# tphakala/birdnet-go

Measured on AMD Instinct MI355X. Metric: 3s-48kHz clips/sec (whole node) + max-abs prob diff vs TFLite, BirdNET v2.4, higher is better.
Workload: dtype f32; 1 GPU; BASELINE configs[1]: BirdNET v2.4 fp32, batch 256 x 3 s @ 48 kHz per GPU, mel front-end + CNN + head on device, raw logits out; batch_per_gpu=256, n_samples=144000, n_classes=6522, pipeline_depth=2, input_sets=4

## Files before the change

### birdnet-go_amd/csrc/engine.cpp

```cpp
#include "engine.h"

#include <algorithm>
#include <cmath>
#include <cstdio>
#include <cstdlib>
#include <cstring>
#include <mutex>
#include <sstream>

#include "../../include/bnhip.h"
#include "hostpipe.h"

namespace bnhip {

#define HIPCHK(call)                                                                           \
    do {                                                                                       \
        hipError_t e_ = (call);                                                                \
        if (e_ != hipSuccess) {                                                                \
            *err = std::string(#call) + ": " + hipGetErrorString(e_);                          \
            return false;                                                                      \
        }                                                                                      \
    } while (0)

Engine::~Engine() {
// ... 154 lines not shown
    return t;
}
bool Engine::tail_taken(int si, int n, bool lane_tuning) const {
    const Step& s = steps[si];
    if (s.kind != S_PW || !s.tail || !s.wbx) return false;
    const int wm = lane_tuning ? s.wm : s.wm_full, nt = lane_tuning ? s.nt : s.nt_full;
    if (wm < 13) return false;
    const int last = si + (s.tail == 1 ? 2 : 1), s_end = part_s1 < 0 ? (int)steps.size() : part_s1;
    if (si < part_s0 || last >= s_end) return false;
    if (s.tail == 2 && steps[si + 1].dwl) return false;
    const PwParams p = pw_params(s, n, lane_tuning);
    if (!pw_tail_ok(p, tail_of(s, steps[si + 1]), nt, wm)) return false;
    return (pw_sw & PW_SW_TAIL_FORCE) || pw_tail_fills(p, nt, wm);
}

float* Engine::vptr(int v, const float* d_in, float* d_logits, float* d_emb, int lane) const {
    if (v < 0) return nullptr;
    if (v == v_input) return const_cast<float*>(d_in);
    if (v == v_logits) return d_logits;
    if (part_hand && v == v_hand) return part_hand;
    (void)d_emb;
    char* base = cur_arena ? cur_arena : act_arena;
    if (lane >= 0) return reinterpret_cast<float*>(base + (size_t)lane * lane_bytes + vals[v].offset_lane);
    return reinterpret_cast<float*>(base + vals[v].offset);
}

hipEvent_t Engine::get_event() {
    if (!ev_pool.empty()) { hipEvent_t e = ev_pool.back(); ev_pool.pop_back(); return e; }
    hipEvent_t e; hipEventCreate(&e); return e;
}
// ... 8 lines not shown
    if (depth <= 1 || (profiling && profile_filter.empty())) return run(d_in, n, d_logits, d_emb, err);
    const int c = (int)(call_idx++ % (unsigned)depth);
    if (ctx_stream[c] != stream) {
        hipEventRecord(ev_ctx_fork, stream);
        hipStreamWaitEvent(ctx_stream[c], ev_ctx_fork, 0);
    }
    cur_arena = ctx_arena[c];
    cur_stream = ctx_stream[c];
    cur_ctx = c;
    bool ok = run_eager(d_in, n, d_logits, d_emb, err);
    cur_arena = nullptr;
    cur_stream = nullptr;
    cur_ctx = -1;
    return ok;
}
bool Engine::run_on_context(int c, hipStream_t st, const float* d_in, int n, float* d_logits, float* d_emb, std::string* err) {
    if (n <= 0 || n > max_batch) { *err = "batch size out of range"; return false; }
    if (c < 0 || c >= kMaxDepth || !st || !ctx_arena[c]) { *err = "context does not exist"; return false; }
    call_idx++;
    cur_arena = ctx_arena[c];
    cur_stream = st;
    cur_ctx = c;
    bool ok = run_eager(d_in, n, d_logits, d_emb, err);
    cur_ctx = -1;
    cur_arena = nullptr;
    cur_stream = nullptr;
    return ok;
}
bool Engine::run_part(int c, hipStream_t st, int s0, int s1, const float* d_in, int n, float* hand, float* d_logits, float* d_emb, std::string* err) {
    if (n <= 0 || n > max_batch) { *err = "batch size out of range"; return false; }
    if (c < 0 || c >= kMaxDepth || !st || !ctx_arena[c]) { *err = "context does not exist"; return false; }
    if (v_hand < 0 || !hand || s0 < 0 || s1 > (int)steps.size() || s0 >= s1 || (s0 != 0 && s0 != split_step) || (s1 != (int)steps.size() && s1 != split_step)) {
        *err = "not a cut of this plan"; return false;
    }
    call_idx++;
    cur_arena = ctx_arena[c];
    cur_stream = st;
    cur_ctx = c;
    part_s0 = s0; part_s1 = s1; part_hand = hand;
    bool ok = run_eager(d_in, n, d_logits, d_emb, err);
    part_s0 = 0; part_s1 = -1; part_hand = nullptr;
    cur_ctx = -1;
    cur_arena = nullptr;
    cur_stream = nullptr;
    return ok;
}
int Engine::heatmap_pruned_step() const {
    if (steps.empty() || precision != 0) return -1;
    const Step& s = steps.back();
    if (s.kind != S_PW || s.out != v_logits || s.in1 >= 0 || s.in2 >= 0 || s.H * s.W != 1 || s.Co != n_classes) return -1;
    if (s.in0 < 0 || vals[s.in0].half || vals[s.in0].elems != (size_t)s.C) return -1;
    return (int)steps.size() - 1;
}
bool Engine::run_head(int s1, const float* d_in, int n, std::string* err) {
    if (n <= 0 || n > max_batch) { *err = "batch size out of range"; return false; }
// ... 40 lines not shown
        }
    }
    if (pick < 0) return;
    split_step = pick; v_hand = crossing[pick];
    if (getenv("BNHIP_DEBUG")) {
        fprintf(stderr, "[bnhip] host split: step %d (%s), value %d (%zu elems/clip%s); candidates:", split_step, steps[split_step].name.c_str(), v_hand,
                vals[v_hand].elems, vals[v_hand].half ? ", bf16" : "");
        for (int k : split_candidates) fprintf(stderr, " %d", k);
        fprintf(stderr, "\n");
    }
}
void Engine::sync_contexts() {
    for (int i = 0; i < kMaxKStreams; i++) if (kstream[i]) hipStreamSynchronize(kstream[i]);
}

bool Engine::run(const float* d_in, int n, float* d_logits, float* d_emb, std::string* err) {
    if (n <= 0 || n > max_batch) { *err = "batch size out of range"; return false; }
    if (call_idx) {
        for (int c = 0; c < kMaxDepth; c++)
            if (ctx_stream[c] && ctx_stream[c] != stream) { hipEventRecord(ev_ctx_done[c], ctx_stream[c]); hipStreamWaitEvent(stream, ev_ctx_done[c], 0); }
        if (kstream[0] && kstream[0] != stream) hipStreamSynchronize(kstream[0]);
    }
    if (!use_graphs || profiling) return run_eager(d_in, n, d_logits, d_emb, err);
    GraphEntry* ge = nullptr;
    for (auto& g : graphs)
        if (g.in == d_in && g.logits == d_logits && g.emb == d_emb && g.n == n) { ge = &g; break; }
    if (ge && ge->exec) {
        hipError_t e = hipGraphLaunch(ge->exec, stream);
        if (e != hipSuccess) { *err = std::string("hipGraphLaunch: ") + hipGetErrorString(e); return false; }
        return true;
    }
    if (!ge) {
        if (graphs.size() >= 8) { if (graphs.front().exec) hipGraphExecDestroy(graphs.front().exec); graphs.erase(graphs.begin()); }
        graphs.push_back(GraphEntry{d_in, d_logits, d_emb, n, 1, nullptr});
        return run_eager(d_in, n, d_logits, d_emb, err);
    }
    hipGraph_t graph = nullptr;
    hipError_t e = hipStreamBeginCapture(stream, hipStreamCaptureModeRelaxed);
    if (e != hipSuccess) { (void)hipGetLastError(); use_graphs = false; return run_eager(d_in, n, d_logits, d_emb, err); }
    bool ok = run_eager(d_in, n, d_logits, d_emb, err);
    e = hipStreamEndCapture(stream, &graph);
    if (!ok || e != hipSuccess || !graph) {
        if (graph) hipGraphDestroy(graph);
        (void)hipGetLastError();
        use_graphs = false;
        return run_eager(d_in, n, d_logits, d_emb, err);
    }
    hipGraphExec_t exec = nullptr;
    e = hipGraphInstantiate(&exec, graph, nullptr, nullptr, 0);
    hipGraphDestroy(graph);
    if (e != hipSuccess || !exec) { (void)hipGetLastError(); use_graphs = false; return run_eager(d_in, n, d_logits, d_emb, err); }
    ge->exec = exec;
    e = hipGraphLaunch(exec, stream);
    if (e != hipSuccess) { *err = std::string("hipGraphLaunch: ") + hipGetErrorString(e); return false; }
    return true;
}

bool Engine::run_eager(const float* d_in_all, int n_all, float* d_logits_all, float* d_emb_all, std::string* err) {
    struct Lane { const float* d_in; int n; float* d_logits; float* d_emb; hipStream_t st; int clip0; };
    Lane lanes[kMaxLanes];
    int nl = 1;
    hipStream_t main_stream = cur_stream ? cur_stream : stream;
    if (mm_dirty) {
        for (int i = 0; i < kMaxKStreams; i++) if (kstream[i]) hipStreamSynchronize(kstream[i]);
        if (stream) hipStreamSynchronize(stream);
        if (mm_scratch) hipMemset(mm_scratch, 0, (size_t)kMaxDepth * kMaxLanes * kMinMaxScratch * sizeof(float));
        (void)hipGetLastError();
        mm_dirty = false;
    }
    if (n_lanes > 1 && !cur_stream && (!profiling || !profile_filter.empty()) && n_all >= dual_lane_min) nl = std::min(n_lanes, n_all);
    for (int li = 0, c0 = 0; li < nl; li++) {
        int cnt = n_all / nl + (li < n_all % nl ? 1 : 0);
        lanes[li] = Lane{d_in_all + (size_t)c0 * n_samples, cnt, d_logits_all + (size_t)c0 * n_classes,
                         d_emb_all ? d_emb_all + (size_t)c0 * emb_dim : nullptr, li == 0 ? main_stream : lane_stream[li - 1], c0};
        c0 += cnt;
    }
    hipEvent_t st_a = nullptr, st_b = nullptr;
    if (step_timing) { hipEventCreate(&st_a); hipEventCreate(&st_b); hipEventRecord(st_a, main_stream); }
    if (nl > 1) {
        hipEventRecord(ev_fork, main_stream);
        for (int li = 1; li < nl; li++) hipStreamWaitEvent(lanes[li].st, ev_fork, 0);
    }
    const int s_end = part_s1 < 0 ? (int)steps.size() : part_s1;
    for (int si = part_s0; si < s_end; si++) {
      for (int li = 0; li < nl; li++) {
        const Step& s = steps[si];
        const float* d_in = lanes[li].d_in; float* d_logits = lanes[li].d_logits; float* d_emb = lanes[li].d_emb;
        const int n = lanes[li].n, clip0 = nl > 1 ? li : -1;
        hipStream_t stream = lanes[li].st;
        float* in0 = vptr(s.in0, d_in, d_logits, d_emb, clip0);
        float* in1 = vptr(s.in1, d_in, d_logits, d_emb, clip0);
        float* in2 = vptr(s.in2, d_in, d_logits, d_emb, clip0);
        float* out = vptr(s.out, d_in, d_logits, d_emb, clip0);
        float* out2 = vptr(s.out2, d_in, d_logits, d_emb, clip0);
        if (s.kind == S_DW && si > 0 && steps[si - 1].tail == 2 && tail_taken(si - 1, n, nl > 1)) continue;
        if (s.kind == S_MEAN_PARTIAL && si > 0 && steps[si - 1].tail == 1 && tail_taken(si - 1, n, nl > 1)) continue;
        if (s.kind == S_MEAN_FINISH && si > 1 && steps[si - 2].tail == 1 && tail_taken(si - 2, n, nl > 1)) continue;
        ProfEntry pe{};
        static const char* dbg_sync_before = getenv("BNHIP_DEBUG_SYNC_BEFORE");
        static const char* dbg_sync_after = getenv("BNHIP_DEBUG_SYNC_AFTER");
        static const char* dbg_ctx1_only = getenv("BNHIP_DEBUG_CTX1_ONLY");
        if (dbg_ctx1_only && cur_ctx == 1 && !strstr(dbg_ctx1_only, s.kclass)) continue;
        static const char* dbg_ctx1_skip = getenv("BNHIP_DEBUG_CTX1_SKIP");
        if (dbg_ctx1_skip && cur_ctx == 1 && strstr(dbg_ctx1_skip, s.kclass)) continue;
        if (dbg_sync_before && (!strcmp(dbg_sync_before, s.kclass) || s.name.rfind(dbg_sync_before, 0) == 0)) hipStreamSynchronize(stream);
        const bool prof_this = profiling && (profile_filter.empty() || profile_filter == s.kclass);
        if (prof_this) { pe.a = get_event(); pe.b = get_event(); pe.step = si; pe.n = n; hipEventRecord(pe.a, stream); }
        switch (s.kind) {
            case S_MINMAX:
                launch_clip_minmax(in0, n, n_samples, specs[0].eps, reinterpret_cast<float2*>(out),
                                   mm_scratch ? mm_scratch + ((size_t)std::max(cur_ctx, 0) * kMaxLanes + (size_t)li) * kMinMaxScratch : nullptr, stream);
                break;
            case S_FRONTEND: {
                const FrontSpec& fs = specs[s.spec];
                FrontendParams p;
                p.x = in0; p.mm = reinterpret_cast<const float2*>(in1); p.G = fs.G; p.window = fs.window; p.out = out;
                p.n_samples = n_samples; p.L = fs.L; p.Lfft = fs.Lfft; p.Kp = fs.Kp; p.hop = fs.hop; p.F = fs.F; p.n_mels = fs.n_mels;
                p.NTP = fs.NTP; p.C = C_spec; p.c = fs.c; p.norm_sub = fs.norm_sub; p.norm_mul = fs.norm_mul;
                p.p1 = fs.p1; p.p2 = fs.p2; p.n_clips = n;
                launch_frontend(p, stream);
                break;
            }
            case S_NORMALIZE:
                launch_normalize(in0, reinterpret_cast<const float2*>(in1), out, n, n_samples, specs[0].norm_sub, specs[0].norm_mul, stream);
// ... 225 lines not shown
}

std::string Engine::profile_read() {
    hipStreamSynchronize(stream);
    struct Agg { double ms = 0, flops = 0, bytes = 0; long launches = 0; };
    std::map<std::string, Agg> agg;
    std::vector<std::string> order;
    std::vector<Agg> per_step(steps.size());
    for (auto& e : prof) {
        float ms = 0;
        hipEventElapsedTime(&ms, e.a, e.b);
        const Step& s = steps[e.step];
        const StepView sv = step_view(*this, e.step);
        if (!agg.count(s.kclass)) order.push_back(s.kclass);
        Agg& a = agg[s.kclass];
        a.ms += ms; a.launches++; a.flops += sv.flops * e.n; a.bytes += sv.bytes * e.n + s.wbytes;
        Agg& ps = per_step[e.step];
        ps.ms += ms; ps.launches++; ps.flops += sv.flops * e.n; ps.bytes += sv.bytes * e.n + s.wbytes;
        ev_pool.push_back(e.a); ev_pool.push_back(e.b);
    }
    prof.clear();
    std::ostringstream os;
    os << "[";
    for (size_t i = 0; i < order.size(); i++) {
        const Agg& a = agg[order[i]];
        os << (i ? "," : "") << "{\"kernel\":\"" << order[i] << "\",\"launches\":" << a.launches << ",\"ms\":" << a.ms
           << ",\"flops\":" << a.flops << ",\"bytes\":" << a.bytes << "}";
    }
    for (size_t i = 0; i < steps.size(); i++) {
        const Agg& a = per_step[i];
        if (!a.launches) continue;
        os << ",{\"step\":" << i << ",\"kernel\":\"" << steps[i].kclass << "\",\"name\":\"";
        jesc(os, step_view(*this, i).name);
// ... 8 lines not shown
```

### birdnet-go_amd/csrc/engine.h

```cpp
#pragma once
#include <hip/hip_runtime.h>

#include <map>
#include <string>
#include <vector>

#include "kernels.h"
#include "tflite_model.h"

namespace bnhip {

enum StepKind { S_MINMAX, S_FRONTEND, S_NORMALIZE, S_STFT, S_MELFIN, S_MELBAND, S_CONV_DIRECT, S_PW, S_DW, S_EXPAND_DW, S_MEAN_PARTIAL, S_MEAN_FINISH, S_SE, S_UNARY, S_BINARY,
                S_EW_UNARY, S_EW_BINARY, S_POOL, S_COPY, S_SOFTMAX, S_REDUCE, S_CONV_GENERIC,
                S_CONV_IGEMM };

struct GenGeom {
    int d[4] = {1, 1, 1, 1};
    long sa[4] = {0, 0, 0, 0}, sb[4] = {0, 0, 0, 0}, so[4] = {0, 0, 0, 0};
    long offa = 0, offo = 0;
    bool a_const = false, b_const = false;
    int mask = 0;
    float alpha = 0.f;
    bool fill = false;
    int dh = 1, dw = 1, depthwise = 0, mult = 1;
// ... 34 lines not shown
    int L, Kp, Lfft, hop, F, n_mels, NTP, c;
    float p1, p2, eps, norm_sub, norm_mul;
    const double* G = nullptr;
    const float* window = nullptr;
    bool fft = false;
    int nb = 0, nbp = 0, mode = 0;
    const float* window_full = nullptr;
    const double* stft_tw = nullptr;
    unsigned stft_zmask = 0xffffffffu;
    const int* bins = nullptr;
    bool normalize = true, log_compress = false, time_major = false;
    int pad_left = 0;
    float log_floor = 0.f, log_scale = 1.f;
};

struct ProfEntry { hipEvent_t a, b; int step; int n; };

struct WeightPlan {
    std::vector<float> img;
    std::vector<size_t> step_w[4];
    std::vector<size_t> step_bx;
};

inline DwParams dw_params(const Step& s, const float* in = nullptr, float* out = nullptr, int n = 1) {
    return DwParams{in, s.w0, s.w1, out, n, s.H, s.W, s.C, s.Ho, s.Wo, s.kh, s.kw, s.sh, s.sw, s.pt, s.pl, s.act};
}
PwTail tail_of(const Step& s, const Step& c);

class Engine {
  public:
    ~Engine();
    bool build(TflModel m, int device, int max_batch, bool plan_only, std::string* err, int* code);
    bool run(const float* d_in, int n, float* d_logits, float* d_emb, std::string* err);

    int device = 0, max_batch = 256;
    bool no_reuse = false;
    bool autotune = true;
    bool defer_weights = false;
    void finish_deferred();
    char* weights_ptr() const { return w_arena; }
    size_t weights_bytes() const { return w_bytes; }
    int frontend_fft = -1;
    int logits_output = -1, embedding_output = -2;
    int precision = 0;
    int bf16x3 = 0;
    int pw_sw = 0;
    bool use_graphs = false;
    void drop_graphs();
    static constexpr int kMaxDepth = 3;
    int depth = 1;
    hipStream_t ctx_stream[kMaxDepth] = {nullptr, nullptr, nullptr};
    char* ctx_arena[kMaxDepth] = {nullptr, nullptr, nullptr};
    static constexpr int kMinMaxScratch = 16 * (2 * kMinMaxParts + 2);
    float* mm_scratch = nullptr;
    bool mm_dirty = false;
    hipEvent_t ev_ctx_fork = nullptr, ev_ctx_done[kMaxDepth] = {nullptr, nullptr, nullptr};
    unsigned call_idx = 0;
    bool run_pipelined(const float* d_in, int n, float* d_logits, float* d_emb, std::string* err);
    void sync_contexts();
    int host_depth = 2;
    bool ensure_contexts(int d, std::string* err, bool with_streams = true);
    bool run_on_context(int c, hipStream_t st, const float* d_in, int n, float* d_logits, float* d_emb, std::string* err);
    int split_step = -1, v_hand = -1;
    float* d_hand = nullptr;
    std::vector<int> split_candidates;
    void pick_split();
    size_t hand_clip_bytes() const { return v_hand < 0 ? 0 : vals[v_hand].elems * (vals[v_hand].half ? 2 : 4); }
    bool ensure_hand(std::string* err);
    bool run_part(int c, hipStream_t st, int s0, int s1, const float* d_in, int n, float* hand, float* d_logits, float* d_emb, std::string* err);
    int heatmap_pruned_step() const;
    bool run_head(int s1, const float* d_in, int n, std::string* err);
    struct HostPipe* hostpipe = nullptr;
    static constexpr int kMaxLanes = 4;
    int n_lanes = 2;
    int dual_lane_min = 32;
    hipStream_t lane_stream[kMaxLanes - 1] = {nullptr, nullptr, nullptr};
    hipEvent_t ev_fork = nullptr, ev_join[kMaxLanes - 1] = {nullptr, nullptr, nullptr};
    void mark_tails();
    bool tail_taken(int si, int n, bool lane_tuning) const;
    PwParams pw_params(const Step& s, int n, bool lane_tuning) const;
    void mark_bf16_storage();
    void tune_or_load();
    void autotune_pw();
    void autotune_expdw();
// ... 34 lines not shown
    float* d_stage_emb = nullptr;
    int16_t* d_stage_pcm = nullptr;
    size_t stage_pcm_bytes = 0;
    float* d_post_conf = nullptr;
    float* d_topk_conf = nullptr;
    int32_t* d_topk_idx = nullptr;
    int topk_cap = 0;

    std::string describe() const;
    std::string profile_read();
    bool step_timing = false;
    std::vector<std::pair<hipEvent_t, hipEvent_t>> step_ev;
    int steps_read(double* start_ms, double* end_ms, int cap);

  private:
    struct GraphEntry { const float* in; float* logits; float* emb; int n; int seen; hipGraphExec_t exec; };
    std::vector<GraphEntry> graphs;
    bool run_eager(const float* d_in, int n, float* d_logits, float* d_emb, std::string* err);
    char* act_arena = nullptr;
    char* cur_arena = nullptr;
    hipStream_t cur_stream = nullptr;
    int cur_ctx = -1;
    int part_s0 = 0, part_s1 = -1;
    float* part_hand = nullptr;
    size_t act_bytes = 0;
    char* w_arena = nullptr;
    size_t w_bytes = 0;
    std::vector<ProfEntry> prof;
    std::vector<hipEvent_t> ev_pool;
    float* vptr(int v, const float* d_in, float* d_logits, float* d_emb, int lane = -1) const;
    int lane_cap = 0;
    size_t lane_bytes = 0;
    hipEvent_t get_event();
// ... 5 lines not shown
```

### birdnet-go_amd/csrc/frontend.hip

```cpp
#include "kernels.h"

#include <cmath>
#include <cstdlib>

namespace bnhip {

__global__ void k_pcm16_to_f32(const int16_t* __restrict__ pcm, float* __restrict__ out, size_t n) {
    size_t i = (size_t)blockIdx.x * blockDim.x + threadIdx.x;
    size_t stride = (size_t)gridDim.x * blockDim.x;
    for (; i < n; i += stride) out[i] = (float)pcm[i] / 32768.0f;
}
__global__ void k_pcm24_to_f32(const uint8_t* __restrict__ pcm, float* __restrict__ out, size_t n) {
    size_t i = (size_t)blockIdx.x * blockDim.x + threadIdx.x;
    size_t stride = (size_t)gridDim.x * blockDim.x;
    for (; i < n; i += stride) {
        int32_t v = (int32_t)pcm[3 * i] | ((int32_t)pcm[3 * i + 1] << 8) | ((int32_t)pcm[3 * i + 2] << 16);
        if (v & 0x00800000) v |= ~0x00FFFFFF;
        out[i] = (float)v / 8388608.0f;
    }
}
__global__ void k_pcm32_to_f32(const int32_t* __restrict__ pcm, float* __restrict__ out, size_t n) {
    size_t i = (size_t)blockIdx.x * blockDim.x + threadIdx.x;
    size_t stride = (size_t)gridDim.x * blockDim.x;
    for (; i < n; i += stride) out[i] = (float)pcm[i] / 2147483648.0f;
// ... 77 lines not shown
                mx = fmaxf(mx, __hip_atomic_load(sc + 2 * g + 1, __ATOMIC_RELAXED, __HIP_MEMORY_SCOPE_AGENT));
            }
            mm[clip] = make_float2(mn, (mx - mn) + eps);
            __hip_atomic_store(cnt, 0u, __ATOMIC_RELAXED, __HIP_MEMORY_SCOPE_AGENT);
        }
    }
}
void launch_clip_minmax(const float* x, int n_clips, int n_samples, float eps, float2* mm, float* scratch, hipStream_t s) {
    if (scratch && n_clips <= 16 && (n_samples & 3) == 0 && n_samples >= 16 * 4096) {
        hipLaunchKernelGGL(k_clip_minmax_parts, dim3(n_clips * kMinMaxParts), dim3(1024), 0, s, x, n_samples, eps, kMinMaxParts, scratch, mm);
        return;
    }
    hipLaunchKernelGGL(k_clip_minmax, dim3(n_clips), dim3(1024), 0, s, x, n_samples, eps, mm);
}

typedef double f64x4 __attribute__((ext_vector_type(4)));
template <int NT, int WN, int FT, int KC>
__global__ __launch_bounds__(64 * (FT / 16) * WN) void k_frontend(FrontendParams p) {
    extern __shared__ __attribute__((aligned(16))) float smem[];
    constexpr int NTP = NT * 16;
    constexpr int NTW = NT / WN;
    constexpr int FG = FT / 16;
    constexpr int NTHR = 64 * FG * WN;
    constexpr int GS = NTP + 16;
    constexpr int GQ = (KC * (NTP / 4) + NTHR - 1) / NTHR;
    const int seg_len = (FT - 1) * p.hop + p.Lfft + 4;
    float* seg = smem;
    float* win = smem + ((seg_len + 3) & ~3);
    float* win2 = win + p.Kp;
    double* Gs = reinterpret_cast<double*>(win2 + p.Kp);
// ... 183 lines not shown
```

### birdnet-go_amd/csrc/hostpipe.cpp

```cpp
#include "hostpipe.h"

#include <cstdint>

#include <hip/hip_runtime.h>

#include <algorithm>
#include <atomic>
#include <chrono>
#include <condition_variable>
#include <cstdio>
#include <cstdlib>
#include <cstring>
#include <deque>
#include <map>
#include <memory>
#include <mutex>
#include <thread>
#include <vector>

#include "../../include/bnhip.h"
#include "engine.h"
#include "numa.h"

namespace bnhip {
// ... 271 lines not shown
    if (j.pcm_bits) {
        const size_t need = (size_t)e.max_batch * e.n_samples * bps;
        if (e.stage_pcm_bytes < need) {
            if (e.d_stage_pcm) { hipStreamSynchronize(e.stream); hipFree(e.d_stage_pcm); e.d_stage_pcm = nullptr; e.stage_pcm_bytes = 0; }
            HP_TRY(hipMalloc((void**)&e.d_stage_pcm, need), "device PCM staging allocation");
            e.stage_pcm_bytes = need;
        }
    }
    for (int off = 0; off < j.n_clips; off += e.max_batch) {
        const int n = std::min(e.max_batch, j.n_clips - off);
        const size_t cnt = (size_t)n * e.n_samples;
        const char* src = (const char*)j.src + (size_t)off * e.n_samples * bps;
        if (j.prepare) j.prepare(off, n);
        if (j.pcm_bits) {
            HP_TRY(hipMemcpyAsync(e.d_stage_pcm, src, cnt * bps, hipMemcpyHostToDevice, e.stream), "H2D copy");
            launch_pcm_to_f32(e.d_stage_pcm, j.pcm_bits, e.d_stage_in, cnt, e.stream);
        } else {
            HP_TRY(hipMemcpyAsync(e.d_stage_in, src, cnt * 4, hipMemcpyHostToDevice, e.stream), "H2D copy");
        }
        if (!e.run(e.d_stage_in, n, e.d_stage_logits, j.emb ? e.d_stage_emb : nullptr, &err)) { hipStreamSynchronize(e.stream); return BNHIP_E_RUNTIME; }
        if (kk) {
            launch_activation(e.d_stage_logits, e.d_post_conf, n, e.n_classes, j.activation, j.sensitivity, e.stream);
            launch_topk(e.d_post_conf, n, e.n_classes, kk, e.d_topk_conf, e.d_topk_idx, e.stream);
            HP_TRY(hipMemcpyAsync(j.out_conf + (size_t)off * kk, e.d_topk_conf, (size_t)n * kk * 4, hipMemcpyDeviceToHost, e.stream), "D2H copy");
            HP_TRY(hipMemcpyAsync(j.out_idx + (size_t)off * kk, e.d_topk_idx, (size_t)n * kk * 4, hipMemcpyDeviceToHost, e.stream), "D2H copy");
        }
        if (j.logits)
            HP_TRY(hipMemcpyAsync(j.logits + (size_t)off * e.n_classes, e.d_stage_logits, (size_t)n * e.n_classes * 4, hipMemcpyDeviceToHost, e.stream), "D2H copy");
        if (j.emb)
            HP_TRY(hipMemcpyAsync(j.emb + (size_t)off * e.emb_dim, e.d_stage_emb, (size_t)n * e.emb_dim * 4, hipMemcpyDeviceToHost, e.stream), "D2H copy");
        HP_TRY(hipStreamSynchronize(e.stream), "synchronize");
    }
    return BNHIP_OK;
}

// ... 125 lines not shown
            if (piecewise && c == 0 && n >= 16) {
                const int pc = (n + 3) / 4;
                for (int q = 0; q < n; q += pc) {
                    const int m = std::min(pc, n - q);
                    j.prepare(cfirst[0] + q, m);
                    HP_PIPE(hipMemcpyAsync(d_dst + (size_t)q * clip_bytes, (const char*)h_src + (size_t)q * clip_bytes, (size_t)m * clip_bytes, hipMemcpyHostToDevice, hp.xfer), "H2D copy");
                }
            } else {
                if (piecewise && c == 0) j.prepare(cfirst[0], n);
                HP_PIPE(hipMemcpyAsync(d_dst, h_src, cnt * bps, hipMemcpyHostToDevice, hp.xfer), "H2D copy");
            }
            HP_PIPE(hipEventRecord(s.ev_h2d, hp.xfer), "event record");
            if (trace) hipEventRecord(tev[1 + 3 * c], hp.xfer);
            HP_PIPE(hipStreamWaitEvent(st, s.ev_h2d, 0), "stream wait");
            if (trace) hipEventRecord(tev[2 + 3 * c], st);
            if (j.pcm_bits) launch_pcm_to_f32(s.d_raw, j.pcm_bits, s.d_in, cnt, st);
            if (!e.run_part(op.st, st, 0, e.split_step, s.d_in, n, reinterpret_cast<float*>(hand + (size_t)cfirst[c] * hcb), s.d_logits, nullptr, &err)) { abort_all(); return BNHIP_E_RUNTIME; }
            HP_PIPE(hipEventRecord(s.ev_comp, st), "event record");
            if (trace) hipEventRecord(tev[3 + 3 * c], st);
            c++;
            if (c < nch) start_fill(c);
        } else {
            HostPipe::Slot& o = hp.s[g];
            const int first = cfirst[gopen], gn = cfirst[c] - first;
            for (int q = gopen; q < c; q++) HP_PIPE(hipStreamWaitEvent(st, hp.s[q % K].ev_comp, 0), "stream wait");
            if (trace) hipEventRecord(tev[1 + 3 * nch + 2 * g], st);
            if (!e.run_part(op.st, st, e.split_step, ns, o.d_in, gn, reinterpret_cast<float*>(hand + (size_t)first * hcb), o.d_logits, j.emb ? o.d_emb : nullptr, &err)) { abort_all(); return BNHIP_E_RUNTIME; }
            if (kk) {
                launch_activation(o.d_logits, o.d_conf, gn, e.n_classes, j.activation, j.sensitivity, st);
                launch_topk(o.d_conf, gn, e.n_classes, kk, o.d_tkc, o.d_tki, st);
            }
            HP_PIPE(hipEventRecord(o.ev_done, st), "event record");
// ... 175 lines not shown
        if (trace) tr.push_back(now_ms() - t_call);
        HostPipe::Slot& s = hp.s[c % K];
        const int n = chunk_n(c), ctx = c % D;
        const size_t cnt = (size_t)n * e.n_samples;
        hipStream_t cs = e.kernel_stream(ctx);
        if (!cs) { abort_all(); err = "hipStreamCreate failed"; return BNHIP_E_RUNTIME; }
        if (!src_pinned) hp.cp->wait(&s.fill);
        if (trace) tr.push_back(now_ms() - t_call);
        const void* h_src = src_pinned ? (const void*)((const char*)j.src + (size_t)cfirst[c] * clip_bytes) : (const void*)s.h_in;
        HP_PIPE(hipMemcpyAsync(j.pcm_bits ? (void*)s.d_raw : (void*)s.d_in, h_src, cnt * bps, hipMemcpyHostToDevice, hp.xfer), "H2D copy");
        HP_PIPE(hipEventRecord(s.ev_h2d, hp.xfer), "event record");
        if (trace) hipEventRecord(tev[1 + 3 * c], hp.xfer);
        if (c >= LAG) HP_PIPE(issue_d2h(c - LAG), "D2H copy");
        HP_PIPE(hipStreamWaitEvent(cs, s.ev_h2d, 0), "stream wait");
        if (trace) hipEventRecord(tev[2 + 3 * c], cs);
        if (j.pcm_bits) launch_pcm_to_f32(s.d_raw, j.pcm_bits, s.d_in, cnt, cs);
        if (!e.run_on_context(ctx, cs, s.d_in, n, s.d_logits, j.emb ? s.d_emb : nullptr, &err)) { abort_all(); return BNHIP_E_RUNTIME; }
        if (kk) {
            launch_activation(s.d_logits, s.d_conf, n, e.n_classes, j.activation, j.sensitivity, cs);
            launch_topk(s.d_conf, n, e.n_classes, kk, s.d_tkc, s.d_tki, cs);
        }
        HP_PIPE(hipEventRecord(s.ev_comp, cs), "event record");
        if (trace) hipEventRecord(tev[3 + 3 * c], cs);
        if (serial) HP_PIPE(hipStreamSynchronize(cs), "synchronize");
        if (trace) tr.push_back(now_ms() - t_call);
        if (c + 1 < nch) HP_PIPE(start_fill(c + 1), "staging");
        if (trace) tr.push_back(now_ms() - t_call);
    }
    for (int c = std::max(0, nch - LAG); c < nch; c++) HP_PIPE(issue_d2h(c), "D2H copy");
    for (int c = std::max(0, nch - K); c < nch; c++) {
        HP_PIPE(finish(hp.s[c % K]), "D2H copy/sync");
        if (trace) fprintf(stderr, "[bnhip] host trace: chunk %d results delivered at %.3f ms\n", c, now_ms() - t_call);
// ... 41 lines not shown
```

### birdnet-go_amd/csrc/kernels.h

```cpp
#pragma once
#include <atomic>
#include <hip/hip_runtime.h>

#include <vector>
#include <cstdint>

namespace bnhip {

inline int device_cus() {
    static std::atomic<int> cus[64];
    int dev = 0;
    if (hipGetDevice(&dev) != hipSuccess) { (void)hipGetLastError(); return 256; }
    if (dev < 0 || dev >= 64) return 256;
    int c = cus[dev].load(std::memory_order_relaxed);
    if (c > 0) return c;
    hipDeviceProp_t pr{};
    if (hipGetDeviceProperties(&pr, dev) != hipSuccess || pr.multiProcessorCount <= 0) { (void)hipGetLastError(); return 256; }
    cus[dev].store(pr.multiProcessorCount, std::memory_order_relaxed);
    return pr.multiProcessorCount;
}

struct PwGrid { int nblk_n; unsigned nblk; };
inline PwGrid pw_grid(int M, int N, int nt, int wm) {
    const int nblk_n = (N + nt * 16 - 1) / (nt * 16);
// ... 8 lines not shown
    if (hipGetDevice(&dev) != hipSuccess) { (void)hipGetLastError(); dev = 0; }
    if (dev < 0 || dev >= 64) { hipFuncSetAttribute(reinterpret_cast<const void*>(Kern), hipFuncAttributeMaxDynamicSharedMemorySize, bytes); return; }
    const unsigned long long bit = 1ull << dev;
    if (done.load(std::memory_order_acquire) & bit) return;
    if (hipFuncSetAttribute(reinterpret_cast<const void*>(Kern), hipFuncAttributeMaxDynamicSharedMemorySize, bytes) == hipSuccess)
        done.fetch_or(bit, std::memory_order_release);
    else (void)hipGetLastError();
}

enum Act : int { ACT_NONE = 0, ACT_RELU = 1, ACT_RELU_N1_TO_1 = 2, ACT_RELU6 = 3, ACT_TANH = 4, ACT_SWISH = 100, ACT_SIGMOID = 101, ACT_HARD_SWISH = 102 };

void launch_pcm_to_f32(const void* pcm, int bits , float* out, size_t n, hipStream_t s);

constexpr int kMinMaxParts = 16;
void launch_clip_minmax(const float* x, int n_clips, int n_samples, float eps, float2* mm, float* scratch , hipStream_t s);

struct FrontendParams {
    const float* x;
    const float2* mm;
    const double* G;
    const float* window;
    float* out;
    int n_samples, L, Lfft, Kp, hop, F, n_mels, NTP, C, c;
    float norm_sub, norm_mul;
    float p1, p2;
    int n_clips;
};
void launch_frontend(const FrontendParams& p, hipStream_t s);
size_t frontend_lds_bytes(int Lfft, int Kp, int hop, int NTP);

// ... 204 lines not shown
```

### birdnet-go_amd/csrc/planner.cpp

```cpp
#include "engine.h"

#include <algorithm>
#include <cmath>
#include <cstdio>
#include <cstdlib>
#include <cstring>
#include <map>

#include "../../include/bnhip.h"

namespace bnhip {

namespace {

size_t align_up(size_t v, size_t a) { return (v + a - 1) / a * a; }

struct Planner {
    const TflModel& m;
    std::vector<int> producer;
    std::vector<std::vector<int>> consumers;
    std::vector<int> uses;
    std::vector<char> absorbed;
    std::string err;

// ... 1431 lines not shown
        p.prec = precision; p.sw = pw_sw;
        int want_wm = 0, want_nt = 6;
        if (const char* e = getenv("BNHIP_PW_TAIL_FORM")) { if (sscanf(e, "%d,%d", &want_wm, &want_nt) != 2) { want_wm = 0; want_nt = 6; } }
        int fit = 0, forced_fit = 0;
        for (int wm : {14, 13, 15}) if (pw_tail_ok(p, t, 6, wm)) { if (!fit) fit = wm; if (wm == want_wm && pw_tail_ok(p, t, want_nt, wm)) forced_fit = wm; }
        if (!fit) continue;
        s.tail = t.kind;
        if (pw_sw & PW_SW_TAIL_FORCE) { s.wm = s.wm_full = forced_fit ? forced_fit : fit; s.nt = s.nt_full = forced_fit ? want_nt : 6; }
    }
}

bool Engine::build(TflModel m, int dev, int maxb, bool plan_only, std::string* err, int* code) {
    device = dev;
    max_batch = maxb;
    pw_sw = pw_switches_from_env();
    const PlanSwitches sw;
    *code = BNHIP_E_UNSUPPORTED;
    if (!run_graph_passes(&m, err)) return false;
    if (!select_outputs(m, &logits_output, &embedding_output)) {
        *code = BNHIP_E_INVALID;
        *err = "logits_output / embedding_output do not name two distinct graph outputs";
        return false;
    }
    Lowering L(*this, m, sw);
    if (!L.input_values() || !L.match_frontends() || !L.frontend() || !L.ops() || !L.bind_outputs()) {
        *err = L.err; *code = L.code;
        return false;
    }
    tensor_value = L.tv;
    mark_tails();

    mark_liveness(vals, steps);
    if (v_emb >= 0) vals[v_emb].last = (int)steps.size();
    for (const Value& v : vals)
        if (v.elems * (size_t)max_batch >= ((size_t)1 << 31)) {
            *err = "max_batch too large for this model: a " + std::to_string(v.elems) + "-element activation times " +
                   std::to_string(max_batch) + " clips exceeds 32-bit indexing";
            *code = BNHIP_E_INVALID;
            return false;
        }
    n_lanes = std::max(1, std::min(n_lanes, kMaxLanes));
    lane_cap = (max_batch + n_lanes - 1) / n_lanes;
    act_bytes = plan_arena(vals, steps, (size_t)max_batch, false, no_reuse);
    lane_bytes = n_lanes > 1 ? align_up(plan_arena(vals, steps, (size_t)lane_cap, true, no_reuse), 256) : 0;
    act_bytes = std::max(act_bytes, lane_bytes * (size_t)n_lanes);
// ... 9 lines not shown
```

Baseline: 77760 clips/s.

## Fuse clip min-max and normalize into one register/LDS-resident kernel with direct PCM input

Adds a kernel that reads each clip once into registers and LDS, computes its min/max, and writes the normalized output. This replaces the separate min-max pass and normalize pass, which each read the clip from memory. When the input is integer PCM and nothing else reads the float input, the kernel also decodes the PCM itself, so the separate pcm-to-f32 conversion kernel and its float write are skipped. The cost is one 1024-thread block per clip with heavy register and LDS use, which may lower occupancy.

```diff
diff --git a/birdnet-go_amd/csrc/engine.cpp b/birdnet-go_amd/csrc/engine.cpp
--- a/birdnet-go_amd/csrc/engine.cpp
+++ b/birdnet-go_amd/csrc/engine.cpp
@@ -192,6 +192,27 @@
     return (pw_sw & PW_SW_TAIL_FORCE) || pw_tail_fills(p, nt, wm);
 }
 
+void Engine::find_norm_pair() {
+    norm_pair = -1; pcm_direct = false;
+    if (!norm_resident || specs.empty()) return;
+    for (int si = 0; si + 1 < (int)steps.size(); si++) {
+        const Step& a = steps[si]; const Step& b = steps[si + 1];
+        if (a.kind == S_MINMAX && b.kind == S_NORMALIZE && a.in0 == v_input && b.in0 == v_input && b.in1 == a.out) { norm_pair = si; break; }
+    }
+    if (norm_pair < 0 || !clip_norm_resident_fits(n_samples)) { norm_pair = -1; return; }
+    pcm_direct = true;
+    for (int si = 0; si < (int)steps.size(); si++) {
+        if (si == norm_pair || si == norm_pair + 1) continue;
+        const Step& s = steps[si];
+        if (s.in0 == v_input || s.in1 == v_input || s.in2 == v_input) pcm_direct = false;
+    }
+}
+bool Engine::norm_resident_taken(int n, const void* x, int bits, const float* xn) const {
+    if (norm_pair < 0 || n <= 16) return false;
+    const uintptr_t in_align = bits == 16 ? 8 : bits == 24 ? 4 : 16;
+    return !(reinterpret_cast<uintptr_t>(x) & (in_align - 1)) && !(reinterpret_cast<uintptr_t>(xn) & 15);
+}
+
 float* Engine::vptr(int v, const float* d_in, float* d_logits, float* d_emb, int lane) const {
     if (v < 0) return nullptr;
     if (v == v_input) return const_cast<float*>(d_in);
@@ -230,31 +251,32 @@
     cur_ctx = -1;
     return ok;
 }
-bool Engine::run_on_context(int c, hipStream_t st, const float* d_in, int n, float* d_logits, float* d_emb, std::string* err) {
+bool Engine::run_on_context(int c, hipStream_t st, const float* d_in, int n, float* d_logits, float* d_emb, std::string* err, PcmSource pcm) {
     if (n <= 0 || n > max_batch) { *err = "batch size out of range"; return false; }
     if (c < 0 || c >= kMaxDepth || !st || !ctx_arena[c]) { *err = "context does not exist"; return false; }
     call_idx++;
     cur_arena = ctx_arena[c];
     cur_stream = st;
     cur_ctx = c;
-    bool ok = run_eager(d_in, n, d_logits, d_emb, err);
+    bool ok = run_eager(d_in, n, d_logits, d_emb, err, pcm);
     cur_ctx = -1;
     cur_arena = nullptr;
     cur_stream = nullptr;
     return ok;
 }
-bool Engine::run_part(int c, hipStream_t st, int s0, int s1, const float* d_in, int n, float* hand, float* d_logits, float* d_emb, std::string* err) {
+bool Engine::run_part(int c, hipStream_t st, int s0, int s1, const float* d_in, int n, float* hand, float* d_logits, float* d_emb, std::string* err, PcmSource pcm) {
     if (n <= 0 || n > max_batch) { *err = "batch size out of range"; return false; }
     if (c < 0 || c >= kMaxDepth || !st || !ctx_arena[c]) { *err = "context does not exist"; return false; }
     if (v_hand < 0 || !hand || s0 < 0 || s1 > (int)steps.size() || s0 >= s1 || (s0 != 0 && s0 != split_step) || (s1 != (int)steps.size() && s1 != split_step)) {
         *err = "not a cut of this plan"; return false;
     }
+    if (pcm.samples && s0 != 0) { *err = "a PCM source belongs to the part that starts the plan"; return false; }
     call_idx++;
     cur_arena = ctx_arena[c];
     cur_stream = st;
     cur_ctx = c;
     part_s0 = s0; part_s1 = s1; part_hand = hand;
-    bool ok = run_eager(d_in, n, d_logits, d_emb, err);
+    bool ok = run_eager(d_in, n, d_logits, d_emb, err, pcm);
     part_s0 = 0; part_s1 = -1; part_hand = nullptr;
     cur_ctx = -1;
     cur_arena = nullptr;
@@ -325,17 +347,17 @@
     for (int i = 0; i < kMaxKStreams; i++) if (kstream[i]) hipStreamSynchronize(kstream[i]);
 }
 
-bool Engine::run(const float* d_in, int n, float* d_logits, float* d_emb, std::string* err) {
+bool Engine::run(const float* d_in, int n, float* d_logits, float* d_emb, std::string* err, PcmSource pcm) {
     if (n <= 0 || n > max_batch) { *err = "batch size out of range"; return false; }
     if (call_idx) {
         for (int c = 0; c < kMaxDepth; c++)
             if (ctx_stream[c] && ctx_stream[c] != stream) { hipEventRecord(ev_ctx_done[c], ctx_stream[c]); hipStreamWaitEvent(stream, ev_ctx_done[c], 0); }
         if (kstream[0] && kstream[0] != stream) hipStreamSynchronize(kstream[0]);
     }
-    if (!use_graphs || profiling) return run_eager(d_in, n, d_logits, d_emb, err);
+    if (!use_graphs || profiling) return run_eager(d_in, n, d_logits, d_emb, err, pcm);
     GraphEntry* ge = nullptr;
     for (auto& g : graphs)
-        if (g.in == d_in && g.logits == d_logits && g.emb == d_emb && g.n == n) { ge = &g; break; }
+        if (g.in == d_in && g.logits == d_logits && g.emb == d_emb && g.n == n && g.pcm == pcm.samples && g.pcm_bits == pcm.bits) { ge = &g; break; }
     if (ge && ge->exec) {
         hipError_t e = hipGraphLaunch(ge->exec, stream);
         if (e != hipSuccess) { *err = std::string("hipGraphLaunch: ") + hipGetErrorString(e); return false; }
@@ -343,31 +365,31 @@
     }
     if (!ge) {
         if (graphs.size() >= 8) { if (graphs.front().exec) hipGraphExecDestroy(graphs.front().exec); graphs.erase(graphs.begin()); }
-        graphs.push_back(GraphEntry{d_in, d_logits, d_emb, n, 1, nullptr});
-        return run_eager(d_in, n, d_logits, d_emb, err);
+        graphs.push_back(GraphEntry{d_in, d_logits, d_emb, n, 1, nullptr, pcm.samples, pcm.bits});
+        return run_eager(d_in, n, d_logits, d_emb, err, pcm);
     }
     hipGraph_t graph = nullptr;
     hipError_t e = hipStreamBeginCapture(stream, hipStreamCaptureModeRelaxed);
-    if (e != hipSuccess) { (void)hipGetLastError(); use_graphs = false; return run_eager(d_in, n, d_logits, d_emb, err); }
-    bool ok = run_eager(d_in, n, d_logits, d_emb, err);
+    if (e != hipSuccess) { (void)hipGetLastError(); use_graphs = false; return run_eager(d_in, n, d_logits, d_emb, err, pcm); }
+    bool ok = run_eager(d_in, n, d_logits, d_emb, err, pcm);
     e = hipStreamEndCapture(stream, &graph);
     if (!ok || e != hipSuccess || !graph) {
         if (graph) hipGraphDestroy(graph);
         (void)hipGetLastError();
         use_graphs = false;
-        return run_eager(d_in, n, d_logits, d_emb, err);
+        return run_eager(d_in, n, d_logits, d_emb, err, pcm);
     }
     hipGraphExec_t exec = nullptr;
     e = hipGraphInstantiate(&exec, graph, nullptr, nullptr, 0);
     hipGraphDestroy(graph);
-    if (e != hipSuccess || !exec) { (void)hipGetLastError(); use_graphs = false; return run_eager(d_in, n, d_logits, d_emb, err); }
+    if (e != hipSuccess || !exec) { (void)hipGetLastError(); use_graphs = false; return run_eager(d_in, n, d_logits, d_emb, err, pcm); }
     ge->exec = exec;
     e = hipGraphLaunch(exec, stream);
     if (e != hipSuccess) { *err = std::string("hipGraphLaunch: ") + hipGetErrorString(e); return false; }
     return true;
 }
 
-bool Engine::run_eager(const float* d_in_all, int n_all, float* d_logits_all, float* d_emb_all, std::string* err) {
+bool Engine::run_eager(const float* d_in_all, int n_all, float* d_logits_all, float* d_emb_all, std::string* err, PcmSource pcm) {
     struct Lane { const float* d_in; int n; float* d_logits; float* d_emb; hipStream_t st; int clip0; };
     Lane lanes[kMaxLanes];
     int nl = 1;
@@ -393,6 +415,17 @@
         for (int li = 1; li < nl; li++) hipStreamWaitEvent(lanes[li].st, ev_fork, 0);
     }
     const int s_end = part_s1 < 0 ? (int)steps.size() : part_s1;
+    const void* res_x[kMaxLanes] = {nullptr, nullptr, nullptr, nullptr};
+    int res_bits[kMaxLanes] = {0, 0, 0, 0};
+    for (int li = 0; li < nl; li++) {
+        const Lane& L = lanes[li];
+        const bool pair_here = norm_pair >= part_s0 && norm_pair + 1 < s_end;
+        const float* xn = pair_here ? vptr(steps[norm_pair + 1].out, L.d_in, L.d_logits, L.d_emb, nl > 1 ? li : -1) : nullptr;
+        const char* src = pcm.samples ? static_cast<const char*>(pcm.samples) + (size_t)L.clip0 * n_samples * (pcm.bits / 8) : nullptr;
+        if (src && pair_here && pcm_direct && norm_resident_taken(L.n, src, pcm.bits, xn)) { res_x[li] = src; res_bits[li] = pcm.bits; continue; }
+        if (src) launch_pcm_to_f32(src, pcm.bits, const_cast<float*>(L.d_in), (size_t)L.n * n_samples, L.st);
+        if (pair_here && norm_resident_taken(L.n, L.d_in, 0, xn)) res_x[li] = L.d_in;
+    }
     for (int si = part_s0; si < s_end; si++) {
       for (int li = 0; li < nl; li++) {
         const Step& s = steps[si];
@@ -407,6 +440,7 @@
         if (s.kind == S_DW && si > 0 && steps[si - 1].tail == 2 && tail_taken(si - 1, n, nl > 1)) continue;
         if (s.kind == S_MEAN_PARTIAL && si > 0 && steps[si - 1].tail == 1 && tail_taken(si - 1, n, nl > 1)) continue;
         if (s.kind == S_MEAN_FINISH && si > 1 && steps[si - 2].tail == 1 && tail_taken(si - 2, n, nl > 1)) continue;
+        if (s.kind == S_NORMALIZE && si == norm_pair + 1 && res_x[li]) continue;
         ProfEntry pe{};
         static const char* dbg_sync_before = getenv("BNHIP_DEBUG_SYNC_BEFORE");
         static const char* dbg_sync_after = getenv("BNHIP_DEBUG_SYNC_AFTER");
@@ -419,6 +453,14 @@
         if (prof_this) { pe.a = get_event(); pe.b = get_event(); pe.step = si; pe.n = n; hipEventRecord(pe.a, stream); }
         switch (s.kind) {
             case S_MINMAX:
+                if (si == norm_pair && res_x[li]) {
+                    if (!launch_clip_norm_resident(res_x[li], res_bits[li], n, n_samples, specs[0].eps, specs[0].norm_sub, specs[0].norm_mul,
+                                                   reinterpret_cast<float2*>(out), vptr(steps[si + 1].out, d_in, d_logits, d_emb, clip0), stream)) {
+                        *err = "k_clip_norm_resident refused a call its predicate accepted"; mm_dirty = true; return false;
+                    }
+                    pe.more_bytes = steps[si + 1].bytes - s.bytes - (res_bits[li] ? (double)n_samples * (4 - res_bits[li] / 8) : 0.0);
+                    break;
+                }
                 launch_clip_minmax(in0, n, n_samples, specs[0].eps, reinterpret_cast<float2*>(out),
                                    mm_scratch ? mm_scratch + ((size_t)std::max(cur_ctx, 0) * kMaxLanes + (size_t)li) * kMinMaxScratch : nullptr, stream);
                 break;
@@ -674,9 +716,9 @@
         const StepView sv = step_view(*this, e.step);
         if (!agg.count(s.kclass)) order.push_back(s.kclass);
         Agg& a = agg[s.kclass];
-        a.ms += ms; a.launches++; a.flops += sv.flops * e.n; a.bytes += sv.bytes * e.n + s.wbytes;
+        a.ms += ms; a.launches++; a.flops += sv.flops * e.n; a.bytes += (sv.bytes + e.more_bytes) * e.n + s.wbytes;
         Agg& ps = per_step[e.step];
-        ps.ms += ms; ps.launches++; ps.flops += sv.flops * e.n; ps.bytes += sv.bytes * e.n + s.wbytes;
+        ps.ms += ms; ps.launches++; ps.flops += sv.flops * e.n; ps.bytes += (sv.bytes + e.more_bytes) * e.n + s.wbytes;
         ev_pool.push_back(e.a); ev_pool.push_back(e.b);
     }
     prof.clear();
diff --git a/birdnet-go_amd/csrc/engine.h b/birdnet-go_amd/csrc/engine.h
--- a/birdnet-go_amd/csrc/engine.h
+++ b/birdnet-go_amd/csrc/engine.h
@@ -72,7 +72,9 @@
     float log_floor = 0.f, log_scale = 1.f;
 };
 
-struct ProfEntry { hipEvent_t a, b; int step; int n; };
+struct PcmSource { const void* samples = nullptr; int bits = 0;  };
+
+struct ProfEntry { hipEvent_t a, b; int step; int n; double more_bytes = 0; };
 
 struct WeightPlan {
     std::vector<float> img;
@@ -89,7 +91,7 @@
   public:
     ~Engine();
     bool build(TflModel m, int device, int max_batch, bool plan_only, std::string* err, int* code);
-    bool run(const float* d_in, int n, float* d_logits, float* d_emb, std::string* err);
+    bool run(const float* d_in, int n, float* d_logits, float* d_emb, std::string* err, PcmSource pcm = {});
 
     int device = 0, max_batch = 256;
     bool no_reuse = false;
@@ -112,20 +114,25 @@
     static constexpr int kMinMaxScratch = 16 * (2 * kMinMaxParts + 2);
     float* mm_scratch = nullptr;
     bool mm_dirty = false;
+    bool norm_resident = true;
+    int norm_pair = -1;
+    bool pcm_direct = false;
+    void find_norm_pair();
+    bool norm_resident_taken(int n, const void* x, int bits, const float* xn) const;
     hipEvent_t ev_ctx_fork = nullptr, ev_ctx_done[kMaxDepth] = {nullptr, nullptr, nullptr};
     unsigned call_idx = 0;
     bool run_pipelined(const float* d_in, int n, float* d_logits, float* d_emb, std::string* err);
     void sync_contexts();
     int host_depth = 2;
     bool ensure_contexts(int d, std::string* err, bool with_streams = true);
-    bool run_on_context(int c, hipStream_t st, const float* d_in, int n, float* d_logits, float* d_emb, std::string* err);
+    bool run_on_context(int c, hipStream_t st, const float* d_in, int n, float* d_logits, float* d_emb, std::string* err, PcmSource pcm = {});
     int split_step = -1, v_hand = -1;
     float* d_hand = nullptr;
     std::vector<int> split_candidates;
     void pick_split();
     size_t hand_clip_bytes() const { return v_hand < 0 ? 0 : vals[v_hand].elems * (vals[v_hand].half ? 2 : 4); }
     bool ensure_hand(std::string* err);
-    bool run_part(int c, hipStream_t st, int s0, int s1, const float* d_in, int n, float* hand, float* d_logits, float* d_emb, std::string* err);
+    bool run_part(int c, hipStream_t st, int s0, int s1, const float* d_in, int n, float* hand, float* d_logits, float* d_emb, std::string* err, PcmSource pcm = {});
     int heatmap_pruned_step() const;
     bool run_head(int s1, const float* d_in, int n, std::string* err);
     struct HostPipe* hostpipe = nullptr;
@@ -190,9 +197,9 @@
     int steps_read(double* start_ms, double* end_ms, int cap);
 
   private:
-    struct GraphEntry { const float* in; float* logits; float* emb; int n; int seen; hipGraphExec_t exec; };
+    struct GraphEntry { const float* in; float* logits; float* emb; int n; int seen; hipGraphExec_t exec; const void* pcm; int pcm_bits; };
     std::vector<GraphEntry> graphs;
-    bool run_eager(const float* d_in, int n, float* d_logits, float* d_emb, std::string* err);
+    bool run_eager(const float* d_in, int n, float* d_logits, float* d_emb, std::string* err, PcmSource pcm = {});
     char* act_arena = nullptr;
     char* cur_arena = nullptr;
     hipStream_t cur_stream = nullptr;
diff --git a/birdnet-go_amd/csrc/frontend.hip b/birdnet-go_amd/csrc/frontend.hip
--- a/birdnet-go_amd/csrc/frontend.hip
+++ b/birdnet-go_amd/csrc/frontend.hip
@@ -1,6 +1,8 @@
 #include "kernels.h"
 
+#include <algorithm>
 #include <cmath>
+#include <cstdint>
 #include <cstdlib>
 
 namespace bnhip {
@@ -115,6 +117,135 @@
     hipLaunchKernelGGL(k_clip_minmax, dim3(n_clips), dim3(1024), 0, s, x, n_samples, eps, mm);
 }
 
+struct Pcm24 {};
+constexpr int kNormR = 28;
+constexpr int kNormRegQuads = 1024 * kNormR;
+constexpr int kNormLdsBytes = 160 * 1024 - 256;
+constexpr int kNormLdsQuads = kNormLdsBytes / 16;
+
+typedef unsigned int u32x2 __attribute__((ext_vector_type(2)));
+typedef unsigned int u32x3 __attribute__((ext_vector_type(3)));
+typedef unsigned int u32x4 __attribute__((ext_vector_type(4)));
+typedef __amdgpu_buffer_rsrc_t ClipBuf;
+__device__ __forceinline__ ClipBuf clip_buf(const void* base, int bytes, int off) {
+    return __builtin_amdgcn_make_buffer_rsrc(const_cast<char*>(static_cast<const char*>(base)) + off, 0, max(bytes - off, 0), 0x00020000);
+}
+template <typename T> struct ClipIn;
+template <> struct ClipIn<float> {
+    static constexpr int kBytes = 4;
+    static __device__ __forceinline__ float4 quad(ClipBuf b, int q) {
+        const u32x4 w = __builtin_amdgcn_raw_buffer_load_b128(b, q * 16, 0, 0);
+        return make_float4(__uint_as_float(w.x), __uint_as_float(w.y), __uint_as_float(w.z), __uint_as_float(w.w));
+    }
+};
+template <> struct ClipIn<int16_t> {
+    static constexpr int kBytes = 2;
+    static __device__ __forceinline__ float s16(uint32_t v) { return (float)(int16_t)v / 32768.0f; }
+    static __device__ __forceinline__ float4 quad(ClipBuf b, int q) {
+        const u32x2 w = __builtin_amdgcn_raw_buffer_load_b64(b, q * 8, 0, 0);
+        return make_float4(s16(w.x), s16(w.x >> 16), s16(w.y), s16(w.y >> 16));
+    }
+};
+template <> struct ClipIn<Pcm24> {
+    static constexpr int kBytes = 3;
+    static __device__ __forceinline__ float s24(uint32_t v) { return (float)((int32_t)(v << 8) >> 8) / 8388608.0f; }
+    static __device__ __forceinline__ float4 quad(ClipBuf b, int q) {
+        const u32x3 w = __builtin_amdgcn_raw_buffer_load_b96(b, q * 12, 0, 0);
+        return make_float4(s24(w.x), s24((w.x >> 24) | (w.y << 8)), s24((w.y >> 16) | (w.z << 16)), s24(w.z >> 8));
+    }
+};
+template <> struct ClipIn<int32_t> {
+    static constexpr int kBytes = 4;
+    static __device__ __forceinline__ float4 quad(ClipBuf b, int q) {
+        const u32x4 w = __builtin_amdgcn_raw_buffer_load_b128(b, q * 16, 0, 0);
+        return make_float4((float)(int32_t)w.x / 2147483648.0f, (float)(int32_t)w.y / 2147483648.0f, (float)(int32_t)w.z / 2147483648.0f,
+                           (float)(int32_t)w.w / 2147483648.0f);
+    }
+};
+__device__ __forceinline__ void quad_minmax(const float4& v, bool in_clip, float& mn, float& mx) {
+    const float a = fminf(fminf(mn, v.x), fminf(v.y, fminf(v.z, v.w)));
+    const float b = fmaxf(fmaxf(mx, v.x), fmaxf(v.y, fmaxf(v.z, v.w)));
+    mn = in_clip ? a : mn;
+    mx = in_clip ? b : mx;
+}
+__device__ __forceinline__ float norm1(float x, float mn, float d, float sub, float mul) {
+    float t = x - mn;
+    t = t / d;
+    t = t - sub;
+    return t * mul;
+}
+__device__ __forceinline__ void store_norm4(ClipBuf o, int q, const float4& v, float mn, float d, float sub, float mul) {
+    u32x4 w;
+    w.x = __float_as_uint(norm1(v.x, mn, d, sub, mul)); w.y = __float_as_uint(norm1(v.y, mn, d, sub, mul));
+    w.z = __float_as_uint(norm1(v.z, mn, d, sub, mul)); w.w = __float_as_uint(norm1(v.w, mn, d, sub, mul));
+    __builtin_amdgcn_raw_buffer_store_b128(w, o, q * 16, 0, 0);
+}
+template <typename T>
+__global__ __launch_bounds__(1024) void k_clip_norm_resident(const void* __restrict__ x, int n_samples, float eps, float norm_sub, float norm_mul,
+                                                             float2* __restrict__ mm, float* __restrict__ out) {
+    extern __shared__ float4 lq[];
+    __shared__ float smn[16], smx[16];
+    constexpr int kIn = ClipIn<T>::kBytes * 4;
+    const char* xc = static_cast<const char*>(x) + (size_t)blockIdx.x * n_samples * ClipIn<T>::kBytes;
+    const float* oc = out + (size_t)blockIdx.x * n_samples;
+    const int n4 = n_samples / 4, nl = max(n4 - kNormRegQuads, 0), tid = threadIdx.x;
+    float mn = INFINITY, mx = -INFINITY;
+    for (int j0 = 0; j0 < nl; j0 += 8 * 1024) {
+        float4 t[8];
+#pragma unroll
+        for (int u = 0; u < 8; u++) t[u] = ClipIn<T>::quad(clip_buf(xc, n4 * kIn, (kNormRegQuads + j0 + u * 1024) * kIn), tid);
+#pragma unroll
+        for (int u = 0; u < 8; u++) {
+            const int j = j0 + u * 1024 + tid;
+            quad_minmax(t[u], j < nl, mn, mx);
+            if (j < nl) lq[j] = t[u];
+        }
+    }
+    float4 v[kNormR];
+#pragma unroll
+    for (int r = 0; r < kNormR; r++) v[r] = ClipIn<T>::quad(clip_buf(xc, n4 * kIn, 1024 * r * kIn), tid);
+#pragma unroll
+    for (int r = 0; r < kNormR; r++) {
+        quad_minmax(v[r], tid + 1024 * r < n4, mn, mx);
+        __builtin_amdgcn_sched_barrier(0);
+    }
+    for (int o = 32; o > 0; o >>= 1) { mn = fminf(mn, __shfl_down(mn, o, 64)); mx = fmaxf(mx, __shfl_down(mx, o, 64)); }
+    if ((tid & 63) == 0) { smn[tid >> 6] = mn; smx[tid >> 6] = mx; }
+    __syncthreads();
+    mn = smn[tid & 15]; mx = smx[tid & 15];
+    for (int o = 8; o > 0; o >>= 1) { mn = fminf(mn, __shfl_xor(mn, o, 16)); mx = fmaxf(mx, __shfl_xor(mx, o, 16)); }
+    const float d = (mx - mn) + eps;
+    if (tid == 0) mm[blockIdx.x] = make_float2(mn, d);
+#pragma unroll
+    for (int r = 0; r < kNormR; r++) {
+        store_norm4(clip_buf(oc, n4 * 16, 1024 * r * 16), tid, v[r], mn, d, norm_sub, norm_mul);
+        __builtin_amdgcn_sched_barrier(0);
+    }
+    const ClipBuf ol = clip_buf(oc, n4 * 16, kNormRegQuads * 16);
+    for (int j = tid; j < nl; j += 1024) store_norm4(ol, j, lq[j], mn, d, norm_sub, norm_mul);
+}
+bool clip_norm_resident_fits(int n_samples) {
+    return n_samples > 0 && (n_samples & 3) == 0 && n_samples / 4 <= kNormRegQuads + kNormLdsQuads;
+}
+template <typename T>
+static void launch_cnr(const void* x, int n_clips, int n_samples, float eps, float norm_sub, float norm_mul, float2* mm, float* out, hipStream_t s) {
+    lds_limit_once<&k_clip_norm_resident<T>>(kNormLdsBytes);
+    const int nl = std::max(n_samples / 4 - kNormRegQuads, 0);
+    hipLaunchKernelGGL(k_clip_norm_resident<T>, dim3(n_clips), dim3(1024), (size_t)nl * 16, s, x, n_samples, eps, norm_sub, norm_mul, mm, out);
+}
+bool launch_clip_norm_resident(const void* x, int bits, int n_clips, int n_samples, float eps, float norm_sub, float norm_mul, float2* mm, float* out,
+                               hipStream_t s) {
+    const uintptr_t in_align = bits == 16 ? 8 : bits == 24 ? 4 : 16;
+    if (n_clips <= 0 || !clip_norm_resident_fits(n_samples) || (reinterpret_cast<uintptr_t>(x) & (in_align - 1)) || (reinterpret_cast<uintptr_t>(out) & 15))
+        return false;
+    if (bits == 0) launch_cnr<float>(x, n_clips, n_samples, eps, norm_sub, norm_mul, mm, out, s);
+    else if (bits == 16) launch_cnr<int16_t>(x, n_clips, n_samples, eps, norm_sub, norm_mul, mm, out, s);
+    else if (bits == 24) launch_cnr<Pcm24>(x, n_clips, n_samples, eps, norm_sub, norm_mul, mm, out, s);
+    else if (bits == 32) launch_cnr<int32_t>(x, n_clips, n_samples, eps, norm_sub, norm_mul, mm, out, s);
+    else return false;
+    return true;
+}
+
 typedef double f64x4 __attribute__((ext_vector_type(4)));
 template <int NT, int WN, int FT, int KC>
 __global__ __launch_bounds__(64 * (FT / 16) * WN) void k_frontend(FrontendParams p) {
diff --git a/birdnet-go_amd/csrc/hostpipe.cpp b/birdnet-go_amd/csrc/hostpipe.cpp
--- a/birdnet-go_amd/csrc/hostpipe.cpp
+++ b/birdnet-go_amd/csrc/hostpipe.cpp
@@ -309,11 +309,11 @@
         if (j.prepare) j.prepare(off, n);
         if (j.pcm_bits) {
             HP_TRY(hipMemcpyAsync(e.d_stage_pcm, src, cnt * bps, hipMemcpyHostToDevice, e.stream), "H2D copy");
-            launch_pcm_to_f32(e.d_stage_pcm, j.pcm_bits, e.d_stage_in, cnt, e.stream);
         } else {
             HP_TRY(hipMemcpyAsync(e.d_stage_in, src, cnt * 4, hipMemcpyHostToDevice, e.stream), "H2D copy");
         }
-        if (!e.run(e.d_stage_in, n, e.d_stage_logits, j.emb ? e.d_stage_emb : nullptr, &err)) { hipStreamSynchronize(e.stream); return BNHIP_E_RUNTIME; }
+        const PcmSource pcm{j.pcm_bits ? e.d_stage_pcm : nullptr, j.pcm_bits};
+        if (!e.run(e.d_stage_in, n, e.d_stage_logits, j.emb ? e.d_stage_emb : nullptr, &err, pcm)) { hipStreamSynchronize(e.stream); return BNHIP_E_RUNTIME; }
         if (kk) {
             launch_activation(e.d_stage_logits, e.d_post_conf, n, e.n_classes, j.activation, j.sensitivity, e.stream);
             launch_topk(e.d_post_conf, n, e.n_classes, kk, e.d_topk_conf, e.d_topk_idx, e.stream);
@@ -469,8 +469,8 @@
             if (trace) hipEventRecord(tev[1 + 3 * c], hp.xfer);
             HP_PIPE(hipStreamWaitEvent(st, s.ev_h2d, 0), "stream wait");
             if (trace) hipEventRecord(tev[2 + 3 * c], st);
-            if (j.pcm_bits) launch_pcm_to_f32(s.d_raw, j.pcm_bits, s.d_in, cnt, st);
-            if (!e.run_part(op.st, st, 0, e.split_step, s.d_in, n, reinterpret_cast<float*>(hand + (size_t)cfirst[c] * hcb), s.d_logits, nullptr, &err)) { abort_all(); return BNHIP_E_RUNTIME; }
+            const PcmSource pcm{j.pcm_bits ? s.d_raw : nullptr, j.pcm_bits};
+            if (!e.run_part(op.st, st, 0, e.split_step, s.d_in, n, reinterpret_cast<float*>(hand + (size_t)cfirst[c] * hcb), s.d_logits, nullptr, &err, pcm)) { abort_all(); return BNHIP_E_RUNTIME; }
             HP_PIPE(hipEventRecord(s.ev_comp, st), "event record");
             if (trace) hipEventRecord(tev[3 + 3 * c], st);
             c++;
@@ -676,8 +676,8 @@
         if (c >= LAG) HP_PIPE(issue_d2h(c - LAG), "D2H copy");
         HP_PIPE(hipStreamWaitEvent(cs, s.ev_h2d, 0), "stream wait");
         if (trace) hipEventRecord(tev[2 + 3 * c], cs);
-        if (j.pcm_bits) launch_pcm_to_f32(s.d_raw, j.pcm_bits, s.d_in, cnt, cs);
-        if (!e.run_on_context(ctx, cs, s.d_in, n, s.d_logits, j.emb ? s.d_emb : nullptr, &err)) { abort_all(); return BNHIP_E_RUNTIME; }
+        const PcmSource pcm{j.pcm_bits ? s.d_raw : nullptr, j.pcm_bits};
+        if (!e.run_on_context(ctx, cs, s.d_in, n, s.d_logits, j.emb ? s.d_emb : nullptr, &err, pcm)) { abort_all(); return BNHIP_E_RUNTIME; }
         if (kk) {
             launch_activation(s.d_logits, s.d_conf, n, e.n_classes, j.activation, j.sensitivity, cs);
             launch_topk(s.d_conf, n, e.n_classes, kk, s.d_tkc, s.d_tki, cs);
diff --git a/birdnet-go_amd/csrc/kernels.h b/birdnet-go_amd/csrc/kernels.h
--- a/birdnet-go_amd/csrc/kernels.h
+++ b/birdnet-go_amd/csrc/kernels.h
@@ -46,6 +46,9 @@
 
 constexpr int kMinMaxParts = 16;
 void launch_clip_minmax(const float* x, int n_clips, int n_samples, float eps, float2* mm, float* scratch , hipStream_t s);
+bool clip_norm_resident_fits(int n_samples);
+bool launch_clip_norm_resident(const void* x, int bits, int n_clips, int n_samples, float eps, float norm_sub, float norm_mul, float2* mm, float* out,
+                               hipStream_t s);
 
 struct FrontendParams {
     const float* x;
diff --git a/birdnet-go_amd/csrc/planner.cpp b/birdnet-go_amd/csrc/planner.cpp
--- a/birdnet-go_amd/csrc/planner.cpp
+++ b/birdnet-go_amd/csrc/planner.cpp
@@ -1469,6 +1469,7 @@
     device = dev;
     max_batch = maxb;
     pw_sw = pw_switches_from_env();
+    if (const char* e = getenv("BNHIP_NORM_RESIDENT")) norm_resident = atoi(e) != 0;
     const PlanSwitches sw;
     *code = BNHIP_E_UNSUPPORTED;
     if (!run_graph_passes(&m, err)) return false;
@@ -1484,6 +1485,7 @@
     }
     tensor_value = L.tv;
     mark_tails();
+    find_norm_pair();
 
     mark_liveness(vals, steps);
     if (v_emb >= 0) vals[v_emb].last = (int)steps.size();
```

Result: faster. 79070 clips/s, median of 6 (+1.7%).
